# KTH-RPL/cloth-splatting

Measured on AMD Instinct MI355X. Metric: rasterizer fwd+bwd rendered Mpix/s (scene_1, 800x800), higher is better.
Workload: dtype f32

## Files before the change

### cloth-splatting_amd/csrc/csplat_raster.hip

```cpp
#include "csplat_common.h"

#include <atomic>
#include <cstring>
#include <chrono>
#include <mutex>
#include <type_traits>

namespace {

constexpr float NEAR_Z = 0.2f;
constexpr int RASTER_MAX_VIEWS = 8;

__device__ constexpr float SH_C0 = 0.28209479177387814f;
__device__ constexpr float SH_C1 = 0.4886025119029199f;
__device__ constexpr float SH_C2[5] = {1.0925484305920792f, -1.0925484305920792f, 0.31539156525252005f,
                                       -1.0925484305920792f, 0.5462742152960396f};
__device__ constexpr float SH_C3[7] = {-0.5900435899266435f, 2.890611442640554f, -0.4570457994644658f,
                                       0.3731763325901154f, -0.4570457994644658f, 1.445305721320277f,
                                       -0.5900435899266435f};

struct Geom {
    float *depth;
    float2 *xy;
    float4 *conic_opacity;
// ... 577 lines not shown
                                                           Cam cam, const uint32_t *__restrict__ table,
                                                           const int2 *__restrict__ ranges, uint64_t *__restrict__ comp) {
    emit_bucket_body(P, tiles, xy, depth, radii, cam, table, ranges, comp);
}

struct P2View {
    Geom g;
    Cam cam;
    const int32_t *radii;
    const uint32_t *table;
    int2 *ranges;
    uint64_t *keys_u, *keys_sorted;
    uint32_t *ids_sorted;
    int *seg_offset, *slot_tile;
    float4 *ckpt;
    uint16_t *mask16;
    unsigned long long *bbits;
    unsigned long long *bmask;
    float4 *recA, *recB;
    float2 *recC;
    const float *bg;
    float *final_T;
    uint32_t *n_contrib;
    float *out_color, *out_depth;
    uint32_t R;
    const uint32_t *info;
    uint32_t Lcap;
    uint32_t Bcap;
    int spec;
};
struct P2Table { P2View v[RASTER_MAX_VIEWS]; uint32_t *valid; int nviews; };
__device__ __forceinline__ bool p2_live(const P2View &w) { return !w.spec || (w.info[0] - 1u < w.R && w.info[1] <= w.Lcap && w.info[2] <= w.Bcap); }
__device__ __forceinline__ void seg_plan_body(int tiles, const int2 *__restrict__ ranges, int *__restrict__ seg_offset,
                                              int *__restrict__ slot_tile);
__global__ __launch_bounds__(BUCKET_G) void k_emit_bucket_views(int P, int tiles, P2Table tab) {
    const P2View &w = tab.v[blockIdx.y];
    if (!p2_live(w)) return;
    if (blockIdx.x == gridDim.x - 1) { seg_plan_body(tiles, w.ranges, w.seg_offset, w.slot_tile); return; }
    emit_bucket_body(P, tiles, w.g.xy, w.g.depth, w.radii, w.cam, w.table, w.ranges, w.keys_u);
}

constexpr int TSORT_THREADS = 1024;
constexpr int TSORT_WAVES = TSORT_THREADS / 64;
constexpr int TSORT_NB = 4 * TSORT_THREADS;
constexpr int TSORT_GRID = 512;
constexpr int TSORT_LONG = 64;
constexpr int TSORT_WORDS = TSORT_NB + 4 + 256 + 8 + 2 + 2 + TSORT_WAVES + 2;
__host__ __device__ inline size_t tsort_lds_bytes(int longest) {
    const int items = (longest > 0 ? longest : 1) + TSORT_THREADS - 1;
    return (size_t)(items / TSORT_THREADS) * TSORT_THREADS * 8 + (size_t)TSORT_WORDS * 4;
}

template <int ITEMS>
__device__ __forceinline__ void tile_sort_body(const int2 *__restrict__ ranges, const uint64_t *__restrict__ comp,
                                               uint64_t *__restrict__ keys_sorted,
                                               uint32_t *__restrict__ ids_sorted, int mode, int tile) {
    extern __shared__ uint64_t s_key[];
    const int2 r = ranges[tile];
    const int n = r.y - r.x;
    if (n <= 0) return;
    const int skip_byte3 = mode & 1;
    const int items = (n + TSORT_THREADS - 1) / TSORT_THREADS;
    uint32_t *s_cnt = reinterpret_cast<uint32_t *>(s_key + (size_t)items * TSORT_THREADS);
    uint32_t *s_dig = s_cnt + TSORT_NB + 4;
    int lane = threadIdx.x & 63, w = threadIdx.x >> 6;
    asm volatile("" : "+v"(lane), "+v"(w));
    const int wbase = w * items * 64;
    const uint64_t lt = (1ull << lane) - 1ull;
    uint64_t key[ITEMS];
    uint32_t rank[ITEMS];
#pragma unroll
    for (int i = 0; i < ITEMS; i++) {
        const int idx = wbase + i * 64 + lane;
        key[i] = (i < items && idx < n) ? comp[r.x + idx] : ~0ull;
    }
    uint32_t *s_diff = s_dig + 264;
    uint32_t *s_mm = s_diff + 2;
    uint32_t *s_wtot = s_mm + 2;
    const uint64_t hi = (uint64_t)(uint32_t)tile << 32;
    if (!(mode & 2)) {
        uint32_t dmin = ~0u, dmax = 0u;
#pragma unroll
        for (int i = 0; i < ITEMS; i++) {
            const int idx = wbase + i * 64 + lane;
            if (i < items && idx < n) { const uint32_t d = (uint32_t)(key[i] >> 32); dmin = min(dmin, d); dmax = max(dmax, d); }
        }
#pragma unroll
        for (int o = 32; o > 0; o >>= 1) {
            dmin = min(dmin, (uint32_t)__shfl_xor((int)dmin, o, 64));
            dmax = max(dmax, (uint32_t)__shfl_xor((int)dmax, o, 64));
        }
        if (threadIdx.x == 0) { s_mm[0] = ~0u; s_mm[1] = 0u; }
        reinterpret_cast<uint4 *>(s_cnt)[threadIdx.x] = make_uint4(0u, 0u, 0u, 0u);
        __syncthreads();
        if (lane == 0) { atomicMin(&s_mm[0], dmin); atomicMax(&s_mm[1], dmax); }
        __syncthreads();
        dmin = s_mm[0]; dmax = s_mm[1];
        if (dmax != dmin) {
            const float scale = (float)TSORT_NB / ((float)(dmax - dmin) + 1.0f);
            uint32_t bs[ITEMS];
#pragma unroll
            for (int i = 0; i < ITEMS; i++) {
                const int idx = wbase + i * 64 + lane;
                if (i < items && idx < n) {
                    const uint32_t b = min((uint32_t)(TSORT_NB - 1), (uint32_t)((float)((uint32_t)(key[i] >> 32) - dmin) * scale));
                    bs[i] = (b << 16) | atomicAdd(&s_cnt[b], 1u);
                }
            }
            __syncthreads();
            const uint4 c = reinterpret_cast<const uint4 *>(s_cnt)[threadIdx.x];
            const uint32_t tot = c.x + c.y + c.z + c.w;
            uint32_t inc = tot;
// ... 15 lines not shown
            const int limit = (mode & 4) ? 1 : TSORT_LONG;
            bool long_run = false;
            uint32_t dst[ITEMS];
#pragma unroll
            for (int i = 0; i < ITEMS; i++) {
                const int idx = wbase + i * 64 + lane;
                if (i < items && idx < n) {
                    const uint32_t b = bs[i] >> 16;
                    const uint32_t lo = s_cnt[b], cb = s_cnt[b + 1] - lo;
                    uint32_t rk = 0;
                    if (cb > (uint32_t)limit) long_run = true;
                    else
#pragma unroll 1
                        for (uint32_t j = 0; j < cb; j++) rk += s_key[lo + j] < key[i] ? 1u : 0u;
                    dst[i] = lo + rk;
                }
            }
            if (!__syncthreads_or(long_run)) {
#pragma unroll
                for (int i = 0; i < ITEMS; i++) {
                    const int idx = wbase + i * 64 + lane;
                    if (i < items && idx < n) s_key[dst[i]] = key[i];
                }
                __syncthreads();
#pragma unroll
                for (int i = 0; i < ITEMS; i++) {
                    const int idx = wbase + i * 64 + lane;
                    if (i < items && idx < n) {
                        const uint64_t k = s_key[idx];
                        keys_sorted[r.x + idx] = hi | (k >> 32);
                        ids_sorted[r.x + idx] = (uint32_t)k;
                    }
                }
                return;
            }
        }
    }
    __syncthreads();
    if (threadIdx.x < 2) s_diff[threadIdx.x] = 0u;
    __syncthreads();
    {
        const uint64_t k0 = comp[r.x];
        uint64_t dv = 0ull;
#pragma unroll
        for (int i = 0; i < ITEMS; i++) {
            const int idx = wbase + i * 64 + lane;
            if (i < items && idx < n) dv |= key[i] ^ k0;
        }
        uint32_t lo = (uint32_t)dv, hi32 = (uint32_t)(dv >> 32);
#pragma unroll
        for (int o = 32; o > 0; o >>= 1) { lo |= (uint32_t)__shfl_xor((int)lo, o, 64); hi32 |= (uint32_t)__shfl_xor((int)hi32, o, 64); }
        if (lane == 0) { atomicOr(&s_diff[0], lo); atomicOr(&s_diff[1], hi32); }
    }
    __syncthreads();
    const uint64_t diffbits = (uint64_t)s_diff[0] | ((uint64_t)s_diff[1] << 32);
    auto pass = [&](int shift) {
        for (int t = threadIdx.x; t < TSORT_WAVES * 256; t += TSORT_THREADS) s_cnt[t] = 0u;
        __syncthreads();
#pragma unroll
        for (int i = 0; i < ITEMS; i++) {
            if (i < items) {
                const int idx = wbase + i * 64 + lane;
                const bool valid = idx < n;
                const uint32_t d = (uint32_t)(key[i] >> shift) & 0xFF;
                unsigned long long peers = __builtin_amdgcn_ballot_w64(valid);
#pragma unroll
                for (int b = 0; b < 8; b++) {
                    const unsigned long long mb = __builtin_amdgcn_ballot_w64(valid && ((d >> b) & 1));
                    peers &= ((d >> b) & 1) ? mb : ~mb;
                }
// ... 56 lines not shown
                const bool starts = (idx == 0 || (uint32_t)(s_key[idx - 1] >> 32) != d) && (uint32_t)(s_key[idx + 1] >> 32) == d;
                if (starts) {
                    int j = idx + 2;
                    while (j < n && j - idx <= TIE_RUN && (uint32_t)(s_key[j] >> 32) == d) j++;
                    if (j - idx > TIE_RUN) long_run = true;
                    else
                        for (int a2 = idx + 1; a2 < j; a2++) {
                            const uint64_t v = s_key[a2];
                            int b2 = a2 - 1;
                            while (b2 >= idx && s_key[b2] > v) { s_key[b2 + 1] = s_key[b2]; b2--; }
                            s_key[b2 + 1] = v;
                        }
                }
            }
        }
        full = __syncthreads_or(long_run);
        if (!full) {
#pragma unroll
            for (int i = 0; i < ITEMS; i++) {
                const int idx = wbase + i * 64 + lane;
                if (i < items && idx < n) key[i] = s_key[idx];
            }
        }
    }
    if (full)
        for (int byte = 0; byte < 8; byte++)
            if (varies(byte)) pass(byte * 8);
#pragma unroll
    for (int i = 0; i < ITEMS; i++) {
        const int idx = wbase + i * 64 + lane;
        if (i < items && idx < n) {
            keys_sorted[r.x + idx] = hi | (key[i] >> 32);
            ids_sorted[r.x + idx] = (uint32_t)key[i];
        }
    }
}
template <int ITEMS, bool DENSE>
__global__ __launch_bounds__(TSORT_THREADS, DENSE ? 8 : 4) void k_tile_sort(const int2 *__restrict__ ranges, const uint64_t *__restrict__ comp,
                                                              uint64_t *__restrict__ keys_sorted,
                                                              uint32_t *__restrict__ ids_sorted, const uint32_t *__restrict__ info, int tiles, int mode) {
    const uint32_t *busy = info + INFO_BUSY, *lpt = busy + tiles + 4;
    const int nbusy = (int)busy[0];
    for (int b = blockIdx.x; b < nbusy; b += gridDim.x) {
        tile_sort_body<ITEMS>(ranges, comp, keys_sorted, ids_sorted, mode, (int)lpt[b]);
        __syncthreads();
    }
}
template <int ITEMS, bool DENSE>
__global__ __launch_bounds__(TSORT_THREADS, DENSE ? 8 : 4) void k_tile_sort_views(P2Table tab, int tiles, int mode) {
    const int lin = blockIdx.y * gridDim.x + blockIdx.x, nv = gridDim.y;
    const P2View &w = tab.v[lin % nv];
    if (!p2_live(w)) return;
    const uint32_t *busy = w.info + INFO_BUSY, *lpt = busy + tiles + 4;
    const int nbusy = (int)busy[0];
    for (int b = lin / nv; b < nbusy; b += gridDim.x) {
        tile_sort_body<ITEMS>(w.ranges, w.keys_u, w.keys_sorted, w.ids_sorted, mode, (int)lpt[b]);
        __syncthreads();
    }
}

template <int CTRL, int RMASK>
__device__ __forceinline__ float dpp_mov(float v, float old) {
    return __int_as_float(__builtin_amdgcn_update_dpp(__float_as_int(old), __float_as_int(v), CTRL, RMASK, 0xF, false));
}
__device__ __forceinline__ float wave_min(float v) {
    v = fminf(v, dpp_mov<0xB1, 0xF>(v, v)); v = fminf(v, dpp_mov<0x4E, 0xF>(v, v));
    v = fminf(v, dpp_mov<0x141, 0xF>(v, v)); v = fminf(v, dpp_mov<0x140, 0xF>(v, v));
    const float r0 = __int_as_float(__builtin_amdgcn_readlane(__float_as_int(v), 0));
    const float r1 = __int_as_float(__builtin_amdgcn_readlane(__float_as_int(v), 16));
    const float r2 = __int_as_float(__builtin_amdgcn_readlane(__float_as_int(v), 32));
    const float r3 = __int_as_float(__builtin_amdgcn_readlane(__float_as_int(v), 48));
    return fminf(fminf(r0, r1), fminf(r2, r3));
}
__device__ __forceinline__ float wave_max(float v) { return -wave_min(-v); }

__device__ __forceinline__ bool box_hit(float2 c, float cut2, float4 co, float bx0, float bx1, float by0, float by1, bool exact) {
    const float lx = bx0 - c.x, hx = bx1 - c.x, ly = by0 - c.y, hy = by1 - c.y;
    const float ex = fmaxf(lx, fminf(0.f, hx)), ey = fmaxf(ly, fminf(0.f, hy));
    if (!(ex * ex + ey * ey <= cut2)) return false;
    if (!exact || cut2 > 1.0e30f) return true;
    const float A = co.x, B = co.y, C = co.z;
    float qmin = 0.f, sabs = 0.f;
    if (ex != 0.f || ey != 0.f) {
        float q1 = 3.0e38f, s1 = 0.f, q2 = 3.0e38f, s2 = 0.f;
        if (ex != 0.f) {
            const float dy = fminf(fmaxf(-B * ex * __builtin_amdgcn_rcpf(fmaxf(C, 1e-30f)), ly), hy);
            const float t0 = A * ex * ex, t1 = 2.f * B * ex * dy, t2 = C * dy * dy;
            q1 = t0 + t1 + t2; s1 = t0 + fabsf(t1) + t2;
        }
        if (ey != 0.f) {
            const float dx = fminf(fmaxf(-B * ey * __builtin_amdgcn_rcpf(fmaxf(A, 1e-30f)), lx), hx);
            const float t0 = C * ey * ey, t1 = 2.f * B * ey * dx, t2 = A * dx * dx;
            q2 = t0 + t1 + t2; s2 = t0 + fabsf(t1) + t2;
        }
        const bool first = q1 <= q2;
        qmin = first ? q1 : q2; sabs = first ? s1 : s2;
    }
    const float tau = 2.f * __logf(255.f * co.w);
    return qmin - 1e-5f * sabs <= tau * 1.001f + 1e-3f;
}

#ifndef CSPLAT_SEG
#define CSPLAT_SEG 256
#endif
constexpr int SEG = CSPLAT_SEG;

__device__ __forceinline__ void seg_plan_body(int tiles, const int2 *__restrict__ ranges, int *__restrict__ seg_offset,
                                              int *__restrict__ slot_tile) {
    __shared__ int s_w[17];
    const int lane = threadIdx.x & 63, w = threadIdx.x >> 6;
    int carry = 0;
    for (int base = 0; base < tiles; base += 1024) {
        const int t = base + threadIdx.x;
        int ns = 0;
        if (t < tiles) { const int2 r = ranges[t]; ns = (r.y - r.x + SEG - 1) / SEG; }
        int inc = ns;
#pragma unroll
        for (int d = 1; d < 64; d <<= 1) { const int o = __shfl_up(inc, d, 64); if (lane >= d) inc += o; }
        if (lane == 63) s_w[w] = inc;
        __syncthreads();
        if (w == 0) {
            int v = lane < 16 ? s_w[lane] : 0, vi = v;
#pragma unroll
            for (int d = 1; d < 16; d <<= 1) { const int o = __shfl_up(vi, d, 64); if (lane >= d) vi += o; }
            if (lane < 16) s_w[lane] = vi - v;
            if (lane == 15) s_w[16] = vi;
        }
        __syncthreads();
        const int ex = carry + s_w[w] + inc - ns;
        if (t < tiles) {
            seg_offset[t] = ex;
            for (int k = 0; k < ns; k++) slot_tile[ex + k] = t;
        }
        carry += s_w[16];
        __syncthreads();
    }
    if (threadIdx.x == 0) seg_offset[tiles] = carry;
}
__global__ __launch_bounds__(1024) void k_seg_plan(int tiles, const int2 *__restrict__ ranges, int *__restrict__ seg_offset,
                                                    int *__restrict__ slot_tile) {
    seg_plan_body(tiles, ranges, seg_offset, slot_tile);
}
__global__ __launch_bounds__(1024) void k_seg_plan_views(int tiles, P2Table tab) {
    const P2View &w = tab.v[blockIdx.x];
    if (!p2_live(w)) return;
    seg_plan_body(tiles, w.ranges, w.seg_offset, w.slot_tile);
}

constexpr float T_EPS = 0.0001f;
constexpr float ALPHA_MIN = 1.f / 255.f;

struct Row4 { float v0, v1, v2, v3; };
__device__ __forceinline__ Row4 rows_allgather(float f) {
    const auto s16 = __builtin_amdgcn_permlane16_swap(__float_as_uint(f), __float_as_uint(f), false, false);
    const auto ev = __builtin_amdgcn_permlane32_swap(s16[0], s16[0], false, false);
    const auto od = __builtin_amdgcn_permlane32_swap(s16[1], s16[1], false, false);
    return {__uint_as_float(ev[0]), __uint_as_float(od[0]), __uint_as_float(ev[1]), __uint_as_float(od[1])};
}
__device__ __forceinline__ float rows_sum(float f) { const Row4 g = rows_allgather(f); return ((g.v0 + g.v1) + g.v2) + g.v3; }
__device__ __forceinline__ float rowsel(int, float a, float b, float c, float d) {
    int x = __float_as_int(a);
    x = __builtin_amdgcn_update_dpp(x, __float_as_int(b), 0xE4, 0x2, 0xF, false);
    x = __builtin_amdgcn_update_dpp(x, __float_as_int(c), 0xE4, 0x4, 0xF, false);
    x = __builtin_amdgcn_update_dpp(x, __float_as_int(d), 0xE4, 0x8, 0xF, false);
    return __int_as_float(x);
}

__device__ __forceinline__ void block_masks_body(int64_t R, int64_t null_at, int gx, const uint64_t *__restrict__ keys_sorted,
                                                 const uint32_t *__restrict__ ids_sorted, const float4 *__restrict__ pack,
                                                 uint16_t *__restrict__ mask16, float4 *__restrict__ recA,
                                                 float4 *__restrict__ recB, float2 *__restrict__ recC, int exact, int64_t block,
                                                 unsigned long long *__restrict__ bmask) {
    const int64_t i = block * 256 + threadIdx.x;
    if (block * 256 > (R | 63) && !(block * 256 <= null_at && null_at < block * 256 + 256)) return;
    if (i == null_at) {
        mask16[i] = 0;
        recA[i] = make_float4(0.f, 0.f, 0.f, 0.f); recB[i] = make_float4(0.f, 0.f, 0.f, 0.f); recC[i] = make_float2(0.f, 0.f);
    }
    uint32_t m = 0;
// ... 1960 lines not shown
    e.det = k.det; e.acc = k.acc;
}

struct Mailboxes {
    volatile uint32_t *host = nullptr;
    uint32_t *dev = nullptr;
    std::atomic<uint32_t> next{1};
    bool tried = false;
};
Mailboxes g_mail;
std::mutex g_mail_mu;
constexpr int MAIL_SLOTS = 64, MAIL_WORDS = 16;

bool mail_init() {
    std::lock_guard<std::mutex> lk(g_mail_mu);
    if (!g_mail.tried) {
        g_mail.tried = true;
        void *h = nullptr, *d = nullptr;
        if (hipHostMalloc(&h, MAIL_SLOTS * MAIL_WORDS * 4, hipHostMallocMapped | hipHostMallocPortable) == hipSuccess &&
            hipHostGetDevicePointer(&d, h, 0) == hipSuccess) {
            memset(h, 0, MAIL_SLOTS * MAIL_WORDS * 4);
            g_mail.host = (volatile uint32_t *)h;
            g_mail.dev = (uint32_t *)d;
        }
        (void)hipGetLastError();
    }
    return g_mail.host != nullptr;
}

unsigned g_debug_flags = 0;
unsigned long long *g_stamp_buf = nullptr;
size_t g_stamp_words = 0;

int tsort_mode(int P) { return (P < (1 << 24) ? 1 : 0) | ((g_debug_flags & 2048u) ? 2 : 0) | ((g_debug_flags & 4096u) ? 4 : 0); }

int higher_msb(uint32_t n) {
    int b = 0;
    while ((1u << b) < n && b < 31) b++;
    return b == 0 ? 1 : b;
}

hipEvent_t pooled_event() {
    constexpr int N = 256;
    static hipEvent_t ring[N];
    static std::atomic<unsigned> next{0};
    static std::mutex mu;
    const unsigned k = next.fetch_add(1) % N;
    std::lock_guard<std::mutex> lk(mu);
    if (!ring[k] && hipEventCreateWithFlags(&ring[k], hipEventDisableTiming) != hipSuccess) { (void)hipGetLastError(); return nullptr; }
    return ring[k];
}

}

extern "C" {

int csplat_abi_version(void) { return CSPLAT_ABI_VERSION; }
int csplat_debug_flags(unsigned flags) { g_debug_flags = flags; return 0; }
unsigned csplat_debug_flags_query(void) { return g_debug_flags; }
int csplat_debug_stamps(void *buf, size_t bytes) { g_stamp_buf = (unsigned long long *)buf; g_stamp_words = bytes / 8; return 0; }
}
unsigned long long *csplat_stamp_buffer(size_t need_words) { return (g_stamp_buf && g_stamp_words >= need_words) ? g_stamp_buf : nullptr; }
extern "C" {
const char *csplat_last_error(void) { return g_csplat_err; }

size_t csplat_geom_bytes(int P) { size_t off[G_NFIELDS]; return geom_offsets(P, off); }
// ... 252 lines not shown
            HIP_TRY(hipMemcpyAsync(host_info, t.info, 12, hipMemcpyDeviceToHost, s));
            HIP_TRY(hipStreamSynchronize(s));
        }
    } else if (t.P > 0) {
        ProfScope ps(PROF_K2, s);
        if (int rc = csplat_inclusive_scan_u32(s, t.g.tiles_touched, t.g.offsets, t.P, t.g.scan_tmp)) return rc;
        HIP_TRY(hipMemcpyAsync(host_info, t.g.offsets + (t.P - 1), 4, hipMemcpyDeviceToHost, s));
        HIP_TRY(hipStreamSynchronize(s));
        host_info[1] = 0xFFFFFFFFu;
        host_info[2] = 0xFFFFFFFFu;
    }
    CSPLAT_REQUIRE(host_info[0] <= 0x7FFFFFFFu, "csplat_forward: more than 2^31 - 1 tile instances (Gaussian x tile pairs) in one view");
    return 0;
}
#define TSORT_FOR_ITEMS(X) X(2) X(4) X(6) X(8)
static int tsort_items(uint32_t longest) {
    const uint32_t items = (longest + TSORT_THREADS - 1) / TSORT_THREADS;
    return items <= 2 ? 2 : items <= 4 ? 4 : items <= 6 ? 6 : 8;
}
static bool tsort_dense(int items, uint64_t busy) {
    static int s_cus = 0;
    if (s_cus <= 0) {
        int dev = 0;
        if (hipGetDevice(&dev) != hipSuccess || hipDeviceGetAttribute(&s_cus, hipDeviceAttributeMultiprocessorCount, dev) != hipSuccess || s_cus <= 0)
            s_cus = 256;
        (void)hipGetLastError();
    }
    return items <= 6 && 2 * busy > 5 * (uint64_t)s_cus;
}
static uint32_t tile_sort_cap() {
    static int s_lds_big = -1;
    if (s_lds_big < 0) {
        bool ok = true;
#define X(I) ok = ok && hipFuncSetAttribute((const void *)k_tile_sort<I, false>, hipFuncAttributeMaxDynamicSharedMemorySize, 96 * 1024) == hipSuccess && \
                  hipFuncSetAttribute((const void *)k_tile_sort<I, I <= 6>, hipFuncAttributeMaxDynamicSharedMemorySize, 96 * 1024) == hipSuccess &&  \
                  hipFuncSetAttribute((const void *)k_tile_sort_views<I, false>, hipFuncAttributeMaxDynamicSharedMemorySize, 96 * 1024) == hipSuccess && \
                  hipFuncSetAttribute((const void *)k_tile_sort_views<I, I <= 6>, hipFuncAttributeMaxDynamicSharedMemorySize, 96 * 1024) == hipSuccess;
        TSORT_FOR_ITEMS(X)
#undef X
        s_lds_big = ok;
        (void)hipGetLastError();
    }
    return s_lds_big ? (uint32_t)BUCKET_CAP : 5120u;
}
static void tile_sort_launch(hipStream_t s, int tiles, uint32_t longest, uint32_t busy, const int2 *ranges, const uint64_t *comp,
                             uint64_t *keys_sorted, uint32_t *ids_sorted, const uint32_t *info, int mode) {
    const size_t lds = tsort_lds_bytes((int)longest);
    const int grid = tiles < TSORT_GRID ? tiles : TSORT_GRID, items = tsort_items(longest);
    const bool dense = tsort_dense(items, busy);
    switch (items) {
#define X(I) case I:                                                                                                                        \
        if (dense) k_tile_sort<I, I <= 6><<<grid, TSORT_THREADS, lds, s>>>(ranges, comp, keys_sorted, ids_sorted, info, tiles, mode);       \
        else k_tile_sort<I, false><<<grid, TSORT_THREADS, lds, s>>>(ranges, comp, keys_sorted, ids_sorted, info, tiles, mode);              \
        break;
        TSORT_FOR_ITEMS(X)
#undef X
    }
}
static void tile_sort_views_launch(hipStream_t s, int tiles, int V, uint32_t Lcap, uint32_t Bcap, const P2Table &tab, int mode) {
    const size_t lds = tsort_lds_bytes((int)Lcap);
    const dim3 grid(tiles < TSORT_GRID ? tiles : TSORT_GRID, V);
    const int items = tsort_items(Lcap);
    const bool dense = tsort_dense(items, (uint64_t)V * (Bcap < (uint32_t)tiles ? Bcap : (uint32_t)tiles));
    switch (items) {
#define X(I) case I:                                                                                           \
        if (dense) k_tile_sort_views<I, I <= 6><<<grid, TSORT_THREADS, lds, s>>>(tab, tiles, mode);            \
        else k_tile_sort_views<I, false><<<grid, TSORT_THREADS, lds, s>>>(tab, tiles, mode);                   \
        break;
        TSORT_FOR_ITEMS(X)
#undef X
    }
}

struct SpecHist { int W = 0, H = 0, P = 0; uint32_t R = 0, longest = 0, busy = 0; };
constexpr int SPEC_RING = 8;
static SpecHist g_spec_ring[SPEC_RING];
static int g_spec_next = 0;
static std::mutex g_spec_mu;

struct PendingViews {
    bool used = false;
    const csplat_view *key = nullptr;
    int V = 0, tk[RASTER_MAX_VIEWS];
    uint32_t Rcap[RASTER_MAX_VIEWS], Lcap = 0, Bcap = 0;
};
constexpr int MAX_PENDING = 8;
static PendingViews g_pending[MAX_PENDING];
static std::mutex g_pending_mu;

static int p2_launch(int V, const int *tk, csplat_view *v, hipStream_t join, const uint32_t *Rcap, uint32_t Lcap, int spec, uint32_t Bcap,
                     uint32_t *valid = nullptr) {
    const FwdTicket &a = g_tickets[tk[0]];
    const int P = a.P, W = a.W, H = a.H, tiles = a.tiles, nb = a.nb;
    {
        P2Table tab;
        tab.valid = valid; tab.nviews = V;
        uint32_t maxR = 0;
        for (int i = 0; i < V; i++) {
            const FwdTicket &t = g_tickets[tk[i]];
            const uint32_t R = Rcap[i];
            maxR = R > maxR ? R : maxR;
            void *bbase = t.alloc(t.alloc_ctx, CSPLAT_CHUNK_BINNING, csplat_binning_bytes(R, W, H));
            void *tbase = t.alloc(t.alloc_ctx, CSPLAT_CHUNK_TEMP, csplat_temp_bytes(P, R, W, H));
            CSPLAT_REQUIRE(bbase && tbase, "allocator returned NULL");
            const BinView b = binning_view(bbase, R, tiles);
            P2View &k = tab.v[i];
            k.g = t.g; k.cam = t.cam; k.radii = t.radii; k.table = t.table; k.ranges = t.ranges;
            k.keys_u = temp_view(tbase, R).keys_u;
            k.keys_sorted = b.keys_sorted; k.ids_sorted = b.ids_sorted; k.seg_offset = b.seg_offset; k.slot_tile = b.slot_tile;
            k.ckpt = b.ckpt; k.mask16 = b.mask16; k.bbits = b.bbits; k.bmask = b.bmask; k.recA = b.recA; k.recB = b.recB; k.recC = b.recC;
            k.bg = t.bg; k.final_T = t.final_T; k.n_contrib = t.n_contrib; k.out_color = v[i].out_color; k.out_depth = v[i].out_depth;
            k.R = R; k.info = t.info; k.Lcap = Lcap; k.Bcap = Bcap; k.spec = spec;
            v[i].layout_rendered = (int)R; v[i].geom = t.gbase; v[i].binning = bbase; v[i].image = t.ibase;
        }
        {
            ProfScope ps(PROF_K3, join);
            k_emit_bucket_views<<<dim3(nb + 1, V), BUCKET_G, (size_t)tiles * 4, join>>>(P, tiles, tab);
            LAUNCH_CHECK();
        }
        {
            ProfScope ps(PROF_K4, join);
            tile_sort_views_launch(join, tiles, V, Lcap, Bcap, tab, tsort_mode(P));
            LAUNCH_CHECK();
        }
        {
            ProfScope ps(PROF_K5, join);
            const int exact = (g_debug_flags & (1u | 16u | 32u)) ? 0 : 1, nbm = cdiv((int64_t)maxR + 1, 256);
            if (V == 1 || V == 2 || V == 4 || V == 8)
                k_block_masks_views<<<dim3((unsigned)(((int64_t)nbm * V + 7) / 8 * 8)), 256, 0, join>>>(tab, exact, V);
            else
                k_block_masks_views<<<dim3(nbm, V), 256, 0, join>>>(tab, exact, 0);
            LAUNCH_CHECK();
        }
        {
            ProfScope ps(PROF_K6, join);
            const int total = cdiv(tiles, 8) * 128, bg_ = cdiv((int)Bcap, 8) * 128, busy_grid = bg_ < total ? bg_ : total;
            if (!(g_debug_flags & 32768u))
                k_composite_fwd_views<false><<<dim3(busy_grid + K6_EXTRA, V), 64, 0, join>>>(tiles, W, H, tab, busy_grid);
            else
                k_composite_fwd_views<true><<<dim3(busy_grid + K6_EXTRA, V), 64, 0, join>>>(tiles, W, H, tab, busy_grid);
            LAUNCH_CHECK();
        }
        return 0;
    }
}

static int finish_views_batched(int V, const int *tk, csplat_view *v, hipStream_t join, bool *done, int mode = 0,
                                PendingViews *pend = nullptr, int *relaunched = nullptr) {
    *done = false;
    if (V < 1 || V > RASTER_MAX_VIEWS || (g_debug_flags & 512u)) return 0;
    const FwdTicket &a = g_tickets[tk[0]];
    for (int i = 0; i < V; i++) {
        const FwdTicket &t = g_tickets[tk[i]];
        if (!t.can_bucket || t.P != a.P || t.W != a.W || t.H != a.H || t.P <= 0) return 0;
    }
    const int P = a.P, W = a.W, H = a.H, tiles = a.tiles;
    const uint32_t cap = tile_sort_cap();
    uint32_t info[RASTER_MAX_VIEWS][3];
    bool have_info = false;
    auto read_counts = [&]() -> int {
// ... 80 lines not shown
    return 0;
}

int csplat_forward_finish(int ticket, float *out_color, float *out_depth, int *num_rendered, void **geom_out,
                          void **binning_out, void **image_out) {
    CSPLAT_REQUIRE(ticket >= 0 && ticket < MAX_TICKETS && g_tickets[ticket].used, "csplat_forward_finish: unknown ticket");
    const FwdTicket t = g_tickets[ticket];
    {
        std::lock_guard<std::mutex> lk(g_ticket_mu);
        g_tickets[ticket].used = false;
    }
    hipStream_t s = t.s;
    const int P = t.P, W = t.W, H = t.H, tiles = t.tiles, nb = t.nb;
    const bool can_bucket = t.can_bucket;
    const Cam cam = t.cam;
    const Geom g = t.g;
    void *gbase = t.gbase, *ibase = t.ibase;
    int2 *ranges = t.ranges;
    uint32_t *n_contrib = t.n_contrib, *table = t.table;
    float *final_T = t.final_T;
    const float *bg = t.bg;
    int32_t *radii = t.radii;
    csplat_alloc_fn alloc = t.alloc;
    void *alloc_ctx = t.alloc_ctx;
    uint32_t host_info[3] = {0, 0, 0};
    if (int rc = finish_read(t, host_info)) return rc;
    const uint32_t R = host_info[0];
    const uint32_t cap = tile_sort_cap();
    const bool bucketed = can_bucket && host_info[1] <= cap;
    *num_rendered = (int)R;
    void *bbase = alloc(alloc_ctx, CSPLAT_CHUNK_BINNING, csplat_binning_bytes(R, W, H));
    CSPLAT_REQUIRE(bbase, "allocator returned NULL");
    const BinView b = binning_view(bbase, R, tiles);
    if (R > 0) {
        void *tbase = alloc(alloc_ctx, CSPLAT_CHUNK_TEMP, csplat_temp_bytes(P, R, W, H));
        CSPLAT_REQUIRE(tbase, "allocator returned NULL");
        const TempView tmp = temp_view(tbase, R);
        if (bucketed) {
            {
                ProfScope ps(PROF_K3, s);
                k_emit_bucket<<<nb, BUCKET_G, (size_t)tiles * 4, s>>>(P, tiles, g.xy, g.depth, radii, cam, table, ranges, tmp.keys_u);
                LAUNCH_CHECK();
            }
            ProfScope ps(PROF_K4, s);
            tile_sort_launch(s, tiles, host_info[1], host_info[2], ranges, tmp.keys_u, b.keys_sorted, b.ids_sorted, t.info, tsort_mode(P));
            LAUNCH_CHECK();
        } else {
            if (can_bucket) {
                ProfScope ps(PROF_K2, s);
                if (int rc = csplat_inclusive_scan_u32(s, g.tiles_touched, g.offsets, P, g.scan_tmp)) return rc;
            }
            {
                ProfScope ps(PROF_K3, s);
                k_emit_keys<<<cdiv(P, 256), 256, 0, s>>>(P, g.xy, g.depth, g.offsets, radii, cam, tmp.keys_u, tmp.ids_u);
                LAUNCH_CHECK();
            }
            const int end_bit = 32 + higher_msb((uint32_t)tiles);
            {
                ProfScope ps(PROF_K4, s);
                if (int rc = csplat_sort_pairs(s, tmp.keys_u, tmp.ids_u, b.keys_sorted, b.ids_sorted, tmp.keys_t, tmp.ids_t, R, end_bit, tmp.sort_tmp))
                    return rc;
            }
            {
                ProfScope ps(PROF_K5, s);
                HIP_TRY(hipMemsetAsync(ranges, 0, (size_t)tiles * 8, s));
                k_tile_ranges<<<cdiv(R, 256), 256, 0, s>>>(R, b.keys_sorted, ranges);
                LAUNCH_CHECK();
            }
        }
    }
    {
        ProfScope ps(PROF_K5, s);
        k_seg_plan<<<1, 1024, 0, s>>>(tiles, ranges, b.seg_offset, b.slot_tile);
        LAUNCH_CHECK();
    }
    {
        ProfScope ps(PROF_K5, s);
        k_block_masks<<<cdiv((int64_t)R + 1, 256), 256, 0, s>>>((int64_t)R, cam.gx, b.keys_sorted, b.ids_sorted, g.pack, b.mask16, b.recA, b.recB,
                                                                 b.recC, (g_debug_flags & (1u | 16u | 32u)) ? 0 : 1, b.bmask);
        LAUNCH_CHECK();
    }
    {
        ProfScope ps(PROF_K6, s);
        if (g_debug_flags & 32768u)
            k_composite_fwd<true><<<cdiv(tiles, 8) * 128, 64, 0, s>>>(tiles, W, H, cam.gx, ranges, b.mask16, b.recA, b.recB, b.recC, R, bg, b.seg_offset,
                                                                      b.ckpt, final_T, n_contrib, out_color, out_depth, b.bbits, b.bmask);
        else
            k_composite_fwd<false><<<cdiv(tiles, 8) * 128, 64, 0, s>>>(tiles, W, H, cam.gx, ranges, b.mask16, b.recA, b.recB, b.recC, R, bg, b.seg_offset,
                                                                       b.ckpt, final_T, n_contrib, out_color, out_depth, b.bbits, b.bmask);
        LAUNCH_CHECK();
    }
    *geom_out = gbase; *binning_out = bbase; *image_out = ibase;
    return 0;
}

int csplat_forward(void *stream, int P, int D, int M, const float *bg, int W, int H, const float *means3D,
                   const float *shs, const float *colors_precomp, const float *opacities, const float *scales,
                   float scale_modifier, const float *rotations, const float *cov3D_precomp, const float *view,
                   const float *proj, const float *campos, float tanfovx, float tanfovy, int prefiltered,
                   csplat_alloc_fn alloc, void *alloc_ctx, float *out_color, float *out_depth, int32_t *radii,
                   int *num_rendered, void **geom_out, void **binning_out, void **image_out) {
    int ticket = -1;
    if (int rc = csplat_forward_begin(stream, P, D, M, bg, W, H, means3D, shs, colors_precomp, opacities, scales, scale_modifier,
                                      rotations, cov3D_precomp, view, proj, campos, tanfovx, tanfovy, prefiltered, alloc,
                                      alloc_ctx, radii, &ticket))
        return rc;
    return csplat_forward_finish(ticket, out_color, out_depth, num_rendered, geom_out, binning_out, image_out);
}

// ... 811 lines not shown
```

Measured before the change: 4611.

## Fuse per-record block-mask generation into the per-tile sort kernel

```diff
diff --git a/cloth-splatting_amd/csrc/csplat_raster.hip b/cloth-splatting_amd/csrc/csplat_raster.hip
--- a/cloth-splatting_amd/csrc/csplat_raster.hip
+++ b/cloth-splatting_amd/csrc/csplat_raster.hip
@@ -633,14 +633,21 @@
 struct P2Table { P2View v[RASTER_MAX_VIEWS]; uint32_t *valid; int nviews; };
 __device__ __forceinline__ bool p2_live(const P2View &w) { return !w.spec || (w.info[0] - 1u < w.R && w.info[1] <= w.Lcap && w.info[2] <= w.Bcap); }
 __device__ __forceinline__ void seg_plan_body(int tiles, const int2 *__restrict__ ranges, int *__restrict__ seg_offset,
-                                              int *__restrict__ slot_tile);
+                                              int *__restrict__ slot_tile, unsigned long long *__restrict__ bmask);
 __global__ __launch_bounds__(BUCKET_G) void k_emit_bucket_views(int P, int tiles, P2Table tab) {
     const P2View &w = tab.v[blockIdx.y];
     if (!p2_live(w)) return;
-    if (blockIdx.x == gridDim.x - 1) { seg_plan_body(tiles, w.ranges, w.seg_offset, w.slot_tile); return; }
+    if (blockIdx.x == gridDim.x - 1) { seg_plan_body(tiles, w.ranges, w.seg_offset, w.slot_tile, w.bmask); return; }
     emit_bucket_body(P, tiles, w.g.xy, w.g.depth, w.radii, w.cam, w.table, w.ranges, w.keys_u);
 }
 
+#ifndef CSPLAT_TSORT_MB
+#define CSPLAT_TSORT_MB 4
+#endif
+#ifndef CSPLAT_TSORT_MB_DENSE
+#define CSPLAT_TSORT_MB_DENSE 2
+#endif
+constexpr int TSORT_MB = CSPLAT_TSORT_MB, TSORT_MB_DENSE = CSPLAT_TSORT_MB_DENSE;
 constexpr int TSORT_THREADS = 1024;
 constexpr int TSORT_WAVES = TSORT_THREADS / 64;
 constexpr int TSORT_NB = 4 * TSORT_THREADS;
@@ -652,10 +659,90 @@
     return (size_t)(items / TSORT_THREADS) * TSORT_THREADS * 8 + (size_t)TSORT_WORDS * 4;
 }
 
-template <int ITEMS>
+struct SortMasks {
+    const float4 *pack;
+    uint16_t *mask16;
+    float4 *recA, *recB;
+    float2 *recC;
+    unsigned long long *bmask;
+    int gx, exact;
+};
+__device__ __forceinline__ bool box_hit(float2 c, float cut2, float4 co, float bx0, float bx1, float by0, float by1, bool exact);
+
+template <int ITEMS, int MB>
+__device__ __forceinline__ void tile_sort_masks(const SortMasks &mk, const int2 r, const int n, const int items, const int tile,
+                                                const int lane, const int w, const uint64_t *s_key, unsigned long long *s_T) {
+    const int wbase = w * items * 64;
+    const float x0 = (float)(((uint32_t)tile % (uint32_t)mk.gx) * CSPLAT_TILE), y0 = (float)(((uint32_t)tile / (uint32_t)mk.gx) * CSPLAT_TILE);
+    const bool exact = mk.exact != 0;
+#pragma unroll 1
+    for (int i0 = 0; i0 < items; i0 += MB) {
+        float4 pa[MB], pb[MB], pc[MB];
+#pragma unroll
+        for (int u = 0; u < MB; u++) {
+            const int idx = wbase + (i0 + u) * 64 + lane;
+            pa[u] = pb[u] = pc[u] = make_float4(0.f, 0.f, 0.f, 0.f);
+            if (i0 + u < items && idx < n) {
+                const size_t id = (uint32_t)s_key[idx];
+                pa[u] = mk.pack[3 * id]; pb[u] = mk.pack[3 * id + 1]; pc[u] = mk.pack[3 * id + 2];
+            }
+        }
+#pragma unroll
+        for (int u = 0; u < MB; u++) {
+            __builtin_amdgcn_sched_barrier(0);
+            const int first = wbase + (i0 + u) * 64;
+            if (i0 + u < items && first < n) {
+                const int idx = first + lane;
+                uint32_t m = 0;
+                if (idx < n) {
+                    const float2 c = make_float2(pa[u].x, pa[u].y);
+                    const float4 co = make_float4(pa[u].z, pa[u].w, pb[u].x, pb[u].y);
+                    const float cut = pc[u].z;
+#pragma unroll
+                    for (int by = 0; by < 4; by++)
+#pragma unroll
+                        for (int bx = 0; bx < 4; bx++)
+                            if (box_hit(c, cut, co, x0 + 4.f * bx, x0 + 4.f * bx + 3.f, y0 + 4.f * by, y0 + 4.f * by + 3.f, exact)) m |= 1u << (by * 4 + bx);
+                    const size_t at = (size_t)r.x + idx;
+                    mk.mask16[at] = (uint16_t)m;
+                    mk.recA[at] = pa[u];
+                    mk.recB[at] = pb[u];
+                    mk.recC[at] = make_float2(pc[u].x, pc[u].y);
+                }
+                uint32_t lo = 0u, hi = 0u;
+#define CSPLAT_WORD_TO_LANE(b)                                                                                                      \
+                {                                                                                                                   \
+                    const unsigned long long wb_ = __builtin_amdgcn_ballot_w64((m >> b) & 1u);                                      \
+                     \
+                    asm("s_nop 1\n\tv_writelane_b32 %0, %2, " #b "\n\tv_writelane_b32 %1, %3, " #b                                  \
+                        : "+v"(lo), "+v"(hi) : "s"((uint32_t)wb_), "s"((uint32_t)(wb_ >> 32)));                                     \
+                }
+                CSPLAT_WORD_TO_LANE(0) CSPLAT_WORD_TO_LANE(1) CSPLAT_WORD_TO_LANE(2) CSPLAT_WORD_TO_LANE(3)
+                CSPLAT_WORD_TO_LANE(4) CSPLAT_WORD_TO_LANE(5) CSPLAT_WORD_TO_LANE(6) CSPLAT_WORD_TO_LANE(7)
+                CSPLAT_WORD_TO_LANE(8) CSPLAT_WORD_TO_LANE(9) CSPLAT_WORD_TO_LANE(10) CSPLAT_WORD_TO_LANE(11)
+                CSPLAT_WORD_TO_LANE(12) CSPLAT_WORD_TO_LANE(13) CSPLAT_WORD_TO_LANE(14) CSPLAT_WORD_TO_LANE(15)
+#undef CSPLAT_WORD_TO_LANE
+                if (lane < 16) s_T[(size_t)(first >> 6) * 16 + lane] = ((unsigned long long)hi << 32) | lo;
+            }
+        }
+    }
+    __syncthreads();
+    const int nch = (n + 63) >> 6, sh = r.x & 63, g0 = r.x >> 6, nglob = ((r.y - 1) >> 6) - g0 + 1;
+    for (int j = threadIdx.x; j < nglob * 16; j += TSORT_THREADS) {
+        const int k = j >> 4, b = j & 15;
+        const unsigned long long below = (k >= 1 && k - 1 < nch) ? s_T[(k - 1) * 16 + b] : 0ull, here = k < nch ? s_T[k * 16 + b] : 0ull;
+        const unsigned long long word = sh ? (below >> (64 - sh)) | (here << sh) : here;
+        unsigned long long *dst = mk.bmask + (size_t)(g0 + k) * 16 + b;
+        const long long at = (long long)(g0 + k) * 64;
+        if (at >= r.x && at + 64 <= r.y) *dst = word;
+        else if (word) atomicOr(dst, word);
+    }
+}
+
+template <int ITEMS, int MB>
 __device__ __forceinline__ void tile_sort_body(const int2 *__restrict__ ranges, const uint64_t *__restrict__ comp,
                                                uint64_t *__restrict__ keys_sorted,
-                                               uint32_t *__restrict__ ids_sorted, int mode, int tile) {
+                                               uint32_t *__restrict__ ids_sorted, int mode, int tile, const SortMasks &mk) {
     extern __shared__ uint64_t s_key[];
     const int2 r = ranges[tile];
     const int n = r.y - r.x;
@@ -679,6 +766,7 @@
     uint32_t *s_mm = s_diff + 2;
     uint32_t *s_wtot = s_mm + 2;
     const uint64_t hi = (uint64_t)(uint32_t)tile << 32;
+    bool sorted = false;
     if (!(mode & 2)) {
         uint32_t dmin = ~0u, dmax = 0u;
 #pragma unroll
@@ -760,10 +848,12 @@
                         ids_sorted[r.x + idx] = (uint32_t)k;
                     }
                 }
-                return;
-            }
-        }
-    }
+                if constexpr (MB > 0) sorted = true;
+                else return;
+            }
+        }
+    }
+    if (!sorted) {
     __syncthreads();
     if (threadIdx.x < 2) s_diff[threadIdx.x] = 0u;
     __syncthreads();
@@ -886,29 +976,44 @@
         if (i < items && idx < n) {
             keys_sorted[r.x + idx] = hi | (key[i] >> 32);
             ids_sorted[r.x + idx] = (uint32_t)key[i];
-        }
-    }
-}
-template <int ITEMS, bool DENSE>
+            if constexpr (MB > 0) s_key[idx] = key[i];
+        }
+    }
+    }
+    if constexpr (MB > 0) tile_sort_masks<ITEMS, MB>(mk, r, n, items, tile, lane, w, s_key, reinterpret_cast<unsigned long long *>(s_cnt));
+}
+__device__ __forceinline__ void sort_null_record(const SortMasks &mk, size_t null_at) {
+    if (threadIdx.x == 0) {
+        mk.mask16[null_at] = 0;
+        mk.recA[null_at] = make_float4(0.f, 0.f, 0.f, 0.f); mk.recB[null_at] = make_float4(0.f, 0.f, 0.f, 0.f); mk.recC[null_at] = make_float2(0.f, 0.f);
+    }
+}
+template <int ITEMS, bool DENSE, bool FUSED>
 __global__ __launch_bounds__(TSORT_THREADS, DENSE ? 8 : 4) void k_tile_sort(const int2 *__restrict__ ranges, const uint64_t *__restrict__ comp,
                                                               uint64_t *__restrict__ keys_sorted,
-                                                              uint32_t *__restrict__ ids_sorted, const uint32_t *__restrict__ info, int tiles, int mode) {
+                                                              uint32_t *__restrict__ ids_sorted, const uint32_t *__restrict__ info, int tiles, int mode,
+                                                              SortMasks mk, uint32_t null_at) {
     const uint32_t *busy = info + INFO_BUSY, *lpt = busy + tiles + 4;
     const int nbusy = (int)busy[0];
+    if (FUSED && blockIdx.x == 0) sort_null_record(mk, null_at);
     for (int b = blockIdx.x; b < nbusy; b += gridDim.x) {
-        tile_sort_body<ITEMS>(ranges, comp, keys_sorted, ids_sorted, mode, (int)lpt[b]);
+        tile_sort_body<ITEMS, !FUSED ? 0 : DENSE ? TSORT_MB_DENSE : TSORT_MB>(ranges, comp, keys_sorted, ids_sorted, mode, (int)lpt[b], mk);
         __syncthreads();
     }
 }
-template <int ITEMS, bool DENSE>
-__global__ __launch_bounds__(TSORT_THREADS, DENSE ? 8 : 4) void k_tile_sort_views(P2Table tab, int tiles, int mode) {
+template <int ITEMS, bool DENSE, bool FUSED>
+__global__ __launch_bounds__(TSORT_THREADS, DENSE ? 8 : 4) void k_tile_sort_views(P2Table tab, int tiles, int mode, int exact) {
     const int lin = blockIdx.y * gridDim.x + blockIdx.x, nv = gridDim.y;
     const P2View &w = tab.v[lin % nv];
     if (!p2_live(w)) return;
     const uint32_t *busy = w.info + INFO_BUSY, *lpt = busy + tiles + 4;
     const int nbusy = (int)busy[0];
+    SortMasks mk;
+    mk.pack = w.g.pack; mk.mask16 = w.mask16; mk.recA = w.recA; mk.recB = w.recB; mk.recC = w.recC; mk.bmask = w.bmask;
+    mk.gx = w.cam.gx; mk.exact = exact;
+    if (FUSED && lin / nv == 0) sort_null_record(mk, w.R);
     for (int b = lin / nv; b < nbusy; b += gridDim.x) {
-        tile_sort_body<ITEMS>(w.ranges, w.keys_u, w.keys_sorted, w.ids_sorted, mode, (int)lpt[b]);
+        tile_sort_body<ITEMS, !FUSED ? 0 : DENSE ? TSORT_MB_DENSE : TSORT_MB>(w.ranges, w.keys_u, w.keys_sorted, w.ids_sorted, mode, (int)lpt[b], mk);
         __syncthreads();
     }
 }
@@ -960,14 +1065,23 @@
 constexpr int SEG = CSPLAT_SEG;
 
 __device__ __forceinline__ void seg_plan_body(int tiles, const int2 *__restrict__ ranges, int *__restrict__ seg_offset,
-                                              int *__restrict__ slot_tile) {
+                                              int *__restrict__ slot_tile, unsigned long long *__restrict__ bmask) {
     __shared__ int s_w[17];
     const int lane = threadIdx.x & 63, w = threadIdx.x >> 6;
     int carry = 0;
     for (int base = 0; base < tiles; base += 1024) {
         const int t = base + threadIdx.x;
         int ns = 0;
-        if (t < tiles) { const int2 r = ranges[t]; ns = (r.y - r.x + SEG - 1) / SEG; }
+        if (t < tiles) {
+            const int2 r = ranges[t];
+            ns = (r.y - r.x + SEG - 1) / SEG;
+            if (bmask && r.y > r.x) {
+                ulonglong2 *first = reinterpret_cast<ulonglong2 *>(bmask + (size_t)(r.x >> 6) * 16);
+                ulonglong2 *behind = reinterpret_cast<ulonglong2 *>(bmask + (size_t)(r.y >> 6) * 16);
+#pragma unroll
+                for (int k = 0; k < 8; k++) { first[k] = make_ulonglong2(0ull, 0ull); behind[k] = make_ulonglong2(0ull, 0ull); }
+            }
+        }
         int inc = ns;
 #pragma unroll
         for (int d = 1; d < 64; d <<= 1) { const int o = __shfl_up(inc, d, 64); if (lane >= d) inc += o; }
@@ -992,13 +1106,13 @@
     if (threadIdx.x == 0) seg_offset[tiles] = carry;
 }
 __global__ __launch_bounds__(1024) void k_seg_plan(int tiles, const int2 *__restrict__ ranges, int *__restrict__ seg_offset,
-                                                    int *__restrict__ slot_tile) {
-    seg_plan_body(tiles, ranges, seg_offset, slot_tile);
+                                                    int *__restrict__ slot_tile, unsigned long long *__restrict__ bmask) {
+    seg_plan_body(tiles, ranges, seg_offset, slot_tile, bmask);
 }
 __global__ __launch_bounds__(1024) void k_seg_plan_views(int tiles, P2Table tab) {
     const P2View &w = tab.v[blockIdx.x];
     if (!p2_live(w)) return;
-    seg_plan_body(tiles, w.ranges, w.seg_offset, w.slot_tile);
+    seg_plan_body(tiles, w.ranges, w.seg_offset, w.slot_tile, nullptr);
 }
 
 constexpr float T_EPS = 0.0001f;
@@ -3025,6 +3139,7 @@
 unsigned long long *g_stamp_buf = nullptr;
 size_t g_stamp_words = 0;
 
+bool sort_masks_fused() { return !(g_debug_flags & 8192u); }
 int tsort_mode(int P) { return (P < (1 << 24) ? 1 : 0) | ((g_debug_flags & 2048u) ? 2 : 0) | ((g_debug_flags & 4096u) ? 4 : 0); }
 
 int higher_msb(uint32_t n) {
@@ -3343,40 +3458,47 @@
     static int s_lds_big = -1;
     if (s_lds_big < 0) {
         bool ok = true;
-#define X(I) ok = ok && hipFuncSetAttribute((const void *)k_tile_sort<I, false>, hipFuncAttributeMaxDynamicSharedMemorySize, 96 * 1024) == hipSuccess && \
-                  hipFuncSetAttribute((const void *)k_tile_sort<I, I <= 6>, hipFuncAttributeMaxDynamicSharedMemorySize, 96 * 1024) == hipSuccess &&  \
-                  hipFuncSetAttribute((const void *)k_tile_sort_views<I, false>, hipFuncAttributeMaxDynamicSharedMemorySize, 96 * 1024) == hipSuccess && \
-                  hipFuncSetAttribute((const void *)k_tile_sort_views<I, I <= 6>, hipFuncAttributeMaxDynamicSharedMemorySize, 96 * 1024) == hipSuccess;
+#define Y(I, F) ok = ok && hipFuncSetAttribute((const void *)k_tile_sort<I, false, F>, hipFuncAttributeMaxDynamicSharedMemorySize, 96 * 1024) == hipSuccess && \
+                  hipFuncSetAttribute((const void *)k_tile_sort<I, I <= 6, F>, hipFuncAttributeMaxDynamicSharedMemorySize, 96 * 1024) == hipSuccess &&  \
+                  hipFuncSetAttribute((const void *)k_tile_sort_views<I, false, F>, hipFuncAttributeMaxDynamicSharedMemorySize, 96 * 1024) == hipSuccess && \
+                  hipFuncSetAttribute((const void *)k_tile_sort_views<I, I <= 6, F>, hipFuncAttributeMaxDynamicSharedMemorySize, 96 * 1024) == hipSuccess;
+#define X(I) Y(I, false) Y(I, true)
         TSORT_FOR_ITEMS(X)
 #undef X
+#undef Y
         s_lds_big = ok;
         (void)hipGetLastError();
     }
     return s_lds_big ? (uint32_t)BUCKET_CAP : 5120u;
 }
 static void tile_sort_launch(hipStream_t s, int tiles, uint32_t longest, uint32_t busy, const int2 *ranges, const uint64_t *comp,
-                             uint64_t *keys_sorted, uint32_t *ids_sorted, const uint32_t *info, int mode) {
+                             uint64_t *keys_sorted, uint32_t *ids_sorted, const uint32_t *info, int mode, const SortMasks &mk, uint32_t null_at) {
     const size_t lds = tsort_lds_bytes((int)longest);
     const int grid = tiles < TSORT_GRID ? tiles : TSORT_GRID, items = tsort_items(longest);
-    const bool dense = tsort_dense(items, busy);
+    const bool dense = tsort_dense(items, busy), fused = mk.mask16 != nullptr;
     switch (items) {
 #define X(I) case I:                                                                                                                        \
-        if (dense) k_tile_sort<I, I <= 6><<<grid, TSORT_THREADS, lds, s>>>(ranges, comp, keys_sorted, ids_sorted, info, tiles, mode);       \
-        else k_tile_sort<I, false><<<grid, TSORT_THREADS, lds, s>>>(ranges, comp, keys_sorted, ids_sorted, info, tiles, mode);              \
+        if (fused && dense) k_tile_sort<I, I <= 6, true><<<grid, TSORT_THREADS, lds, s>>>(ranges, comp, keys_sorted, ids_sorted, info, tiles, mode, mk, null_at); \
+        else if (fused) k_tile_sort<I, false, true><<<grid, TSORT_THREADS, lds, s>>>(ranges, comp, keys_sorted, ids_sorted, info, tiles, mode, mk, null_at);      \
+        else if (dense) k_tile_sort<I, I <= 6, false><<<grid, TSORT_THREADS, lds, s>>>(ranges, comp, keys_sorted, ids_sorted, info, tiles, mode, mk, null_at);    \
+        else k_tile_sort<I, false, false><<<grid, TSORT_THREADS, lds, s>>>(ranges, comp, keys_sorted, ids_sorted, info, tiles, mode, mk, null_at);                \
         break;
         TSORT_FOR_ITEMS(X)
 #undef X
     }
 }
-static void tile_sort_views_launch(hipStream_t s, int tiles, int V, uint32_t Lcap, uint32_t Bcap, const P2Table &tab, int mode) {
+static void tile_sort_views_launch(hipStream_t s, int tiles, int V, uint32_t Lcap, uint32_t Bcap, const P2Table &tab, int mode, int fused,
+                                   int exact) {
     const size_t lds = tsort_lds_bytes((int)Lcap);
     const dim3 grid(tiles < TSORT_GRID ? tiles : TSORT_GRID, V);
     const int items = tsort_items(Lcap);
     const bool dense = tsort_dense(items, (uint64_t)V * (Bcap < (uint32_t)tiles ? Bcap : (uint32_t)tiles));
     switch (items) {
 #define X(I) case I:                                                                                           \
-        if (dense) k_tile_sort_views<I, I <= 6><<<grid, TSORT_THREADS, lds, s>>>(tab, tiles, mode);            \
-        else k_tile_sort_views<I, false><<<grid, TSORT_THREADS, lds, s>>>(tab, tiles, mode);                   \
+        if (fused && dense) k_tile_sort_views<I, I <= 6, true><<<grid, TSORT_THREADS, lds, s>>>(tab, tiles, mode, exact);   \
+        else if (fused) k_tile_sort_views<I, false, true><<<grid, TSORT_THREADS, lds, s>>>(tab, tiles, mode, exact);        \
+        else if (dense) k_tile_sort_views<I, I <= 6, false><<<grid, TSORT_THREADS, lds, s>>>(tab, tiles, mode, exact);      \
+        else k_tile_sort_views<I, false, false><<<grid, TSORT_THREADS, lds, s>>>(tab, tiles, mode, exact);                  \
         break;
         TSORT_FOR_ITEMS(X)
 #undef X
@@ -3429,14 +3551,15 @@
             k_emit_bucket_views<<<dim3(nb + 1, V), BUCKET_G, (size_t)tiles * 4, join>>>(P, tiles, tab);
             LAUNCH_CHECK();
         }
+        const int exact = (g_debug_flags & (1u | 16u | 32u)) ? 0 : 1, fused = sort_masks_fused() ? 1 : 0;
         {
             ProfScope ps(PROF_K4, join);
-            tile_sort_views_launch(join, tiles, V, Lcap, Bcap, tab, tsort_mode(P));
+            tile_sort_views_launch(join, tiles, V, Lcap, Bcap, tab, tsort_mode(P), fused, exact);
             LAUNCH_CHECK();
         }
-        {
+        if (!fused) {
             ProfScope ps(PROF_K5, join);
-            const int exact = (g_debug_flags & (1u | 16u | 32u)) ? 0 : 1, nbm = cdiv((int64_t)maxR + 1, 256);
+            const int nbm = cdiv((int64_t)maxR + 1, 256);
             if (V == 1 || V == 2 || V == 4 || V == 8)
                 k_block_masks_views<<<dim3((unsigned)(((int64_t)nbm * V + 7) / 8 * 8)), 256, 0, join>>>(tab, exact, V);
             else
@@ -3583,6 +3706,7 @@
     void *bbase = alloc(alloc_ctx, CSPLAT_CHUNK_BINNING, csplat_binning_bytes(R, W, H));
     CSPLAT_REQUIRE(bbase, "allocator returned NULL");
     const BinView b = binning_view(bbase, R, tiles);
+    bool fused = false;
     if (R > 0) {
         void *tbase = alloc(alloc_ctx, CSPLAT_CHUNK_TEMP, csplat_temp_bytes(P, R, W, H));
         CSPLAT_REQUIRE(tbase, "allocator returned NULL");
@@ -3593,8 +3717,17 @@
                 k_emit_bucket<<<nb, BUCKET_G, (size_t)tiles * 4, s>>>(P, tiles, g.xy, g.depth, radii, cam, table, ranges, tmp.keys_u);
                 LAUNCH_CHECK();
             }
+            if (sort_masks_fused()) {
+                fused = true;
+                ProfScope ps(PROF_K5, s);
+                k_seg_plan<<<1, 1024, 0, s>>>(tiles, ranges, b.seg_offset, b.slot_tile, b.bmask);
+                LAUNCH_CHECK();
+            }
+            SortMasks mk;
+            mk.pack = g.pack; mk.mask16 = fused ? b.mask16 : nullptr; mk.recA = b.recA; mk.recB = b.recB; mk.recC = b.recC; mk.bmask = b.bmask;
+            mk.gx = cam.gx; mk.exact = (g_debug_flags & (1u | 16u | 32u)) ? 0 : 1;
             ProfScope ps(PROF_K4, s);
-            tile_sort_launch(s, tiles, host_info[1], host_info[2], ranges, tmp.keys_u, b.keys_sorted, b.ids_sorted, t.info, tsort_mode(P));
+            tile_sort_launch(s, tiles, host_info[1], host_info[2], ranges, tmp.keys_u, b.keys_sorted, b.ids_sorted, t.info, tsort_mode(P), mk, R);
             LAUNCH_CHECK();
         } else {
             if (can_bucket) {
@@ -3620,12 +3753,12 @@
             }
         }
     }
-    {
+    if (!fused) {
         ProfScope ps(PROF_K5, s);
-        k_seg_plan<<<1, 1024, 0, s>>>(tiles, ranges, b.seg_offset, b.slot_tile);
+        k_seg_plan<<<1, 1024, 0, s>>>(tiles, ranges, b.seg_offset, b.slot_tile, nullptr);
         LAUNCH_CHECK();
     }
-    {
+    if (!fused) {
         ProfScope ps(PROF_K5, s);
         k_block_masks<<<cdiv((int64_t)R + 1, 256), 256, 0, s>>>((int64_t)R, cam.gx, b.keys_sorted, b.ids_sorted, g.pack, b.mask16, b.recA, b.recB,
                                                                  b.recC, (g_debug_flags & (1u | 16u | 32u)) ? 0 : 1, b.bmask);
```

Result: slower. 4226 (-8.4%).
